# ariloytynoja/pagan2-msa

Hardware: AMD Instinct MI355X
Metric: DP cells/sec, 32x100 kb DNA progressive align (hot path in dependency order: fill + traceback per tree level) (higher is better)
Workload: dtype f64; 1 GPU; cfg4_32x100kb_dna_anchored; leaves=32, length=100000, data_type=dna, anchors=prefix, offset 15, node_alignments=31, order=guide-tree levels one after the other (a parent needs its children)

## Files before the change

### pagan2-msa_amd/csrc/dp_pipe.hip

```cpp
#include "dp_kcommon.h"
#include <type_traits>

#define PNW 4
#define PNT (64 * PNW)
#define PNTW PG_PIPE_WIDTH
#define PRK PG_PIPE_RING
#define PAGE PG_PIPE_REACH
#define PRW 512
#define PEC PG_PIPE_EDGE_CAP
#define PDR 128
#define PDR_REACH 60
#define PLOOK 64
#define PLAND 8
#define PNA PG_PIPE_ASSIST
#define PST PG_PIPE_STAGE
#define PBLOCK (PNT + 64 * PNA + 64)
static_assert(PNTW == PNT - PAGE && PRK >= PAGE && PG_PIPE_WINDOW + 80 <= PRW, "kernel geometry out of step with dp_device.h");
static_assert(PNA == 3 && PST == 3 && PAGE >= PLAND + 4, "assist wave a stages the diagonals d % 3 == a into slot a, at most two diagonals ahead; far cells have landed");
#define PFAR_POOL ((PNT * 4) / 24)
#define PS_ONLY 0x80000000u
#define PS_FIRST 0x40000000u
#define PS_BP 0x3fffffffu
#ifndef PG_SPIN_LIMIT_LOG2
#define PG_SPIN_LIMIT_LOG2 25
// ... 2002 lines not shown
            l2q[q] = r2q[q] = lSq[q] = rSq[q] = false;
            int kL = 0, kR = 0;
            gl[q] = pg_i4{0, 0, 0, 0}; gr[q] = pg_i4{0, 0, 0, 0};
#pragma unroll
            for (int t = 0; t < 8; ++t) { o_f[q][t].need = false; o_f[q][t].boff = 0; o_xy[q][t].x = NIw; o_xy[q][t].y = NIw; o_m[q][t] = NIw; }
            if (!__any(r <= hi)) continue;
            if (r <= hi) {
                gl[q] = PM.recL[r & (PRW - 1)]; gr[q] = PM.recR[j & (PRW - 1)];
                const int nl = (gl[q].x >> PR_NE_SHIFT) & 127, nr = (gr[q].x >> PR_NE_SHIFT) & 127;
                const int dl0 = gl[q].y & 0xffff, dl1 = (int)((unsigned)gl[q].y >> 16), dr0 = gr[q].y & 0xffff, dr1 = (int)((unsigned)gr[q].y >> 16);
                const bool easyL = nl == 1 ? dl0 == 1 : (nl == 2 && (dl0 == 1) != (dl1 == 1));
                const bool easyR = nr == 1 ? dr0 == 1 : (nr == 2 && (dr0 == 1) != (dr1 == 1));
                const bool l2 = nl == 2, r2 = nr == 2;
                const bool lS = l2 && dl0 != 1, rS = r2 && dr0 != 1;
                kL = lS ? dl0 : dl1; kR = rS ? dr0 : dr1;
                const bool inner = r >= 2 && r <= Lx - 2 && j >= 2 && j <= Ly - 2 && (!l2 || r - kL >= 1) && (!r2 || j - kR >= 1);
                kind[q] = (easyL && easyR && inner) ? 1 : 2;
                if (kind[q] == 1) { l2q[q] = l2; r2q[q] = r2; lSq[q] = lS; rSq[q] = rS; }
            }
            const bool b1 = kind[q] == 1, l2 = l2q[q], r2 = r2q[q];
            if (!__any(b1 && (l2 || r2))) continue;
            auto rd = [&](bool need, int age, int p_, pg_d2 &xy, double &m) {
                int rb = wsb - age * wrow_bytes;
                rb += rb < 0 ? wk * wrow_bytes : 0;
                const int off = need ? rb + wpos(p_) * 24 : (int)offsetof(PipeSmem, null_cell) - (int)offsetof(PipeSmem, sc);
                const double *c = (const double *)((const char *)&PM.sc[0][0][0] + off);
                xy.x = c[PG_X]; xy.y = c[PG_Y]; m = c[PG_M];
            };
            auto fetch = [&](int t, bool need, int age, int p_) {
                if (!__any(need)) return;
                if (!__any(need && age > amax)) rd(need, age, p_, o_xy[q][t], o_m[q][t]);
                else { o_f[q][t] = wcell(need, age, p_, o_xy[q][t], o_m[q][t]); any_far = true; }
            };
            fetch(3, b1 && l2, kL, r - kL);
            fetch(4, b1 && l2, kL + 1, r - kL);
            fetch(5, b1 && r2, kR, r);
            fetch(6, b1 && r2, kR + 1, r - 1);
            fetch(7, b1 && l2 && r2, kL + kR, r - kL);
        }
#ifdef PG_PIPE_STATS
        const long long st_t2 = __builtin_readcyclecounter();
#endif
        if (any_far) {
            far_fetch8(sc_out, o_f[0], o_xy[0], o_m[0]);
            far_fetch8(sc_out, o_f[1], o_xy[1], o_m[1]);
        }
#ifdef PG_PIPE_STATS
        const long long st_t3 = __builtin_readcyclecounter();
#endif
#pragma unroll
        for (int q = 0; q < 2; ++q) {
            const int r = wrow[q], j = d - r;
            const bool active = kind[q] != 0;
            if (__any(active)) n_now += 2;
            double bx = NIw, by = NIw, bm = NIw;
            unsigned px = PG_BP_NONE, py = PG_BP_NONE, pm = PG_BP_NONE;
            if (kind[q] == 1) {
                const bool l2 = l2q[q], r2 = r2q[q], lS = lSq[q], rS = rSq[q];
                const int ti_ = ((gl[q].x & 0xffff) + __umul24(gr[q].x & 0xffff, S)) & 255;
                const double tM = PM.tab2[ti_][0], tX = PM.tab2[ti_][1];
                const double lw0 = (double)__int_as_float(gl[q].z), lw1 = (double)__int_as_float(gl[q].w);
                const double rw0 = (double)__int_as_float(gr[q].z), rw1 = (double)__int_as_float(gr[q].w);
                const double lwA = lS ? lw1 : lw0, lwS = lS ? lw0 : lw1, rwA = rS ? rw1 : rw0, rwS = rS ? rw0 : rw1;
                const pg_d2 lx_ = o_xy[q][3], lm_ = o_xy[q][4], ry_ = o_xy[q][5], rm_ = o_xy[q][6], lr_ = o_xy[q][7];
                const double lxm = o_m[q][3], lmm = o_m[q][4], rym = o_m[q][5], rmm = o_m[q][6], lrm = o_m[q][7];
                auto gapv = [&](double own, double other, double m_) { return __builtin_fmax(own + ge, __builtin_fmax(other, m_ + ng) + go); };
                auto pairv = [&](double x_, double y_, double m_, double lw, double rw) {
                    return (__builtin_fmax(m_ + tM, __builtin_fmax(x_, y_) + tX) + lw) + rw;
                };
                bx = gapv(Ux[q], Uy[q], Um[q]);
                by = gapv(Py[q], Px[q], Pm[q]);
                bm = pairv(Cx[q], Cy[q], Cm[q], lwA, rwA);
                if (__any(r2)) {
                    by = __builtin_fmax(by, gapv(ry_.y, ry_.x, rym));
                    bm = __builtin_fmax(bm, pairv(rm_.x, rm_.y, rmm, lwA, rwS));
                }
                if (__any(l2)) {
                    bx = __builtin_fmax(bx, gapv(lx_.x, lx_.y, lxm));
                    bm = __builtin_fmax(bm, pairv(lm_.x, lm_.y, lmm, lwS, rwA));
                    if (__any(l2 && r2)) bm = __builtin_fmax(bm, pairv(lr_.x, lr_.y, lrm, lwS, rwS));
                }
            } else if (kind[q] == 2) {
                const int nl = (gl[q].x >> PR_NE_SHIFT) & 127, nr = (gr[q].x >> PR_NE_SHIFT) & 127;
                double tM_ = 0, tX_ = 0;
                if (r > 0 && j > 0 && nl > 0 && nr > 0) {
                    const int ti_ = ((gl[q].x & 0xffff) + __umul24(gr[q].x & 0xffff, S)) & 255;
                    tM_ = PM.tab2[ti_][0]; tX_ = PM.tab2[ti_][1];
                }
                const pg_i4 gl_ = gl[q], gr_ = gr[q];
                cell_any_t(J, r, j, r > 0 ? nl : 0, j > 0 ? nr : 0, tM_, tX_, no_terminal_edges, reduced_terminal,
                         [&](int p_, int q_, double &xs, double &ys, double &ms) {
                             pg_d2 xy; double m_;
                             const FarAsk f = wcell(p_ >= 0 && q_ >= 0, d - (p_ + q_), p_, xy, m_);
                             {
                                 const FarAsk none = {false, 0};
                                 pg_d2 e1 = {NIw, NIw}, e2 = {NIw, NIw}, e3 = {NIw, NIw}; double m1 = NIw, m2 = NIw, m3 = NIw;
                                 far_fetch4(sc_out, f, none, none, none, xy, m_, e1, m1, e2, m2, e3, m3);
                             }
                             xs = xy.x; ys = xy.y; ms = m_;
                         },
                         [&](int k, int &p_, double &lw) { int dist; edge_at<true>(gl_, k, r, dist, lw); p_ = r - dist; },
                         [&](int k, int &q_, double &rw) { int dist; edge_at<false>(gr_, k, j, dist, rw); q_ = j - dist; },
                         bx, by, bm, px, py, pm);
            }
            if (__any(active && ((gl[q].x | gr[q].x) & PR_SRC))) { if (active) hist_append(gl[q], gr[q], r, j, bx, by, bm); }
            if (r < lo + wpos_n) {
                double *o = (double *)((char *)&PM.sc[0][0][0] + wsb + wpos(r) * 24);
                o[PG_X] = bx; o[PG_Y] = by; o[PG_M] = bm;
            }
            if (active) {
                const unsigned off24 = __umul24((unsigned)(r - lo), 24u);
                pg_d2 xy; xy.x = bx; xy.y = by;
                *(PG_GLOBAL pg_d2 *)(srow + off24) = xy;
                *(PG_GLOBAL double *)(srow + off24 + 16u) = bm;
            }
            Px[q] = bx; Py[q] = by; Pm[q] = bm;
            Cx[q] = Ux[q]; Cy[q] = Uy[q]; Cm[q] = Um[q];
        }
        {
            const int tot = n_now + n_hist1 + n_hist2;
            if (tot >= 12) asm volatile("s_waitcnt vmcnt(12)" ::: "memory");
            else if (tot >= 10) asm volatile("s_waitcnt vmcnt(10)" ::: "memory");
            else if (tot >= 8) asm volatile("s_waitcnt vmcnt(8)" ::: "memory");
            else if (tot >= 6) asm volatile("s_waitcnt vmcnt(6)" ::: "memory");
            else if (tot >= 4) asm volatile("s_waitcnt vmcnt(4)" ::: "memory");
            else if (tot >= 2) asm volatile("s_waitcnt vmcnt(2)" ::: "memory");
            else asm volatile("s_waitcnt vmcnt(0)" ::: "memory");
            n_hist2 = n_hist1; n_hist1 = n_now;
        }
        flag_store(&PM.progress[wave], d);
#ifdef PG_PIPE_STATS
        {
            const long long st_t5 = __builtin_readcyclecounter();
            st_cls_t[4] += st_t5 - st_step0; ++st_cls_n[4];
            st_w[0] += st_t1 - st_step0; st_w[1] += st_t2 - st_t1; st_w[2] += st_t3 - st_t2; st_w[3] += st_t5 - st_t3;
        }
#endif
        ++d;
        lo_prev = lo;
        if (d >= run_end || flag_load(&PM.abort_flag) != 0) break;
        cur.x = __builtin_amdgcn_readfirstlane(nxt.x); cur.y = __builtin_amdgcn_readfirstlane(nxt.y);
        cur.z = __builtin_amdgcn_readfirstlane(nxt.z); cur.w = __builtin_amdgcn_readfirstlane(nxt.w);
    }
    dA = psc[d];
    row = dA.x + ((tid - dA.x) & (PNT - 1));
    ok_until = d - 1;
    C_.dA = dA;
    WCTX_OUT(C_);
}

#define PW7 7
#define PW7L (64 * PW7)
static_assert(PW7 == PNW + PNA && PG_PIPE_WINDOW <= PW7L - 16, "seven-wave wide runs: one row per lane");
__device__ __noinline__ void wide_run7(WaveCtx &C_) {
    WCTX_IN(C_);
    WCTX_STATS(C_);
    const PgDevJob *__restrict__ job = (const PgDevJob *)uniform_u64((unsigned long long)C_.job);
    const unsigned flags_ = __builtin_amdgcn_readfirstlane(C_.flags);
    const bool no_terminal_edges = flags_ & 1u, reduced_terminal = !(flags_ & 2u);
    pg_i8 dA = uniform_i8(C_.dA);
    const View J = load_view(job);
    const int d0 = d;
    const int lane = tid & 63, w7 = wave, up7 = w7 == 0 ? PW7 - 1 : w7 - 1;
    const double NIw = neg_inf();
    asm volatile("s_waitcnt vmcnt(0)" ::: "memory");
    flag_store(&PM.wflag[w7], d0 - 1);
    flag_store(&PM.warrived[w7], d0);
    for (int w = 0; w < PW7; ++w) POLLX(&PM.warrived[w], d0, 7);
    p_up = d0 - 1 > p_up ? d0 - 1 : p_up;
    p_dn = d0 - 1 > p_dn ? d0 - 1 : p_dn;
    int run_end = d0 + 1;
    for (;;) {
        const int t = run_end + lane;
        const int c4 = ((PG_GLOBAL const int *)psc)[8 * (t < nd ? t : nd) + 4] & 15;
        const unsigned long long stop = __builtin_amdgcn_ballot_w64(t >= nd || c4 != 4);
        if (stop != 0) { run_end += __builtin_ctzll(stop); break; }
        run_end += 64;
    }
    asm volatile("s_waitcnt vmcnt(0)" ::: "memory");
    pg_i4 cur = {dA.x, dA.y, dA.z, dA.w};
    int wr;
    { int m_ = (tid - cur.x) % PW7L; m_ += m_ < 0 ? PW7L : 0; wr = cur.x + m_; }
    if (diags_ld < d0) diags_ld = POLLX(&PM.loaded[2], d0, 5);
    double Px, Py, Pm, Cx, Cy, Cm, Ux, Uy, Um;
    {
        const FarAsk fP = far_ask(psc, d0, 1, wr), fC = far_ask(psc, d0, 2, wr - 1), fU = far_ask(psc, d0, 1, wr - 1), none = {false, 0};
        pg_d2 a = {NIw, NIw}, b = {NIw, NIw}, c = {NIw, NIw}, e = {NIw, NIw};
        double ma = NIw, mb = NIw, mc = NIw, me = NIw;
        far_fetch4(sc_out, fP, fC, fU, none, a, ma, b, mb, c, mc, e, me);
        Px = a.x; Py = a.y; Pm = ma; Cx = b.x; Cy = b.y; Cm = mb; Ux = c.x; Uy = c.y; Um = mc;
    }
    const bool geo_b = (dA.s4 & 16) != 0;
    const int wpos_n = geo_b ? PWPOS_B : PWPOS_A, wk = geo_b ? PWK_B : PWK_A, wage = wk - 2, wrow_bytes = wpos_n * 24;
    int wbase = cur.x - 32;
    auto wpos = [&](int r_) { int q_ = r_ - wbase; q_ -= q_ >= wpos_n ? wpos_n : 0; q_ -= q_ >= wpos_n ? wpos_n : 0; return q_; };
    int n_hist1 = 0, n_hist2 = 0;
    int lo_prev = cur.x;
    for (;;) {
        const int lo = cur.x, hi = cur.y;
        if (lo - 2 * wage - 4 - wbase >= wpos_n) wbase += wpos_n;
#ifdef PG_PIPE_STATS
        const long long st_step0 = __builtin_readcyclecounter();
#endif
        {
            const int nr_ = hi + 1 < Lx ? hi + 1 : Lx, nc_ = d - lo + 1 < Ly ? d - lo + 1 : Ly;
            if (rows_ld < nr_) rows_ld = POLLX(&PM.loaded[0], nr_, 1);
            if (cols_ld < nc_) cols_ld = POLLX(&PM.loaded[1], nc_, 2);
            if (diags_ld < d) diags_ld = POLLX(&PM.loaded[2], d, 5);
        }
        const int r = wr < lo ? wr + PW7L : wr, j = d - r;
        int kind = 0;
        pg_i4 gl = {0, 0, 0, 0}, gr = {0, 0, 0, 0};
        bool l2 = false, r2 = false, l3 = false, r3 = false;
        int kL = 1, kR = 1, kL3 = 1, kR3 = 1;
        double lwA = 0, lwS = 0, lwT = 0, rwA = 0, rwS = 0, rwT = 0;
        double tM = 0, tX = 0;
        if (r <= hi) {
            gl = PM.recL[r & (PRW - 1)]; gr = PM.recR[j & (PRW - 1)];
            const int nl = (gl.x >> PR_NE_SHIFT) & 127, nr = (gr.x >> PR_NE_SHIFT) & 127;
            auto shape = [&](auto left_tag, const pg_i4 &rec, int site, int n, bool &two, bool &three, int &k1, int &k3, double &wA, double &w1, double &w3) -> bool {
                constexpr bool LEFT = decltype(left_tag)::value;
                const int e0 = rec.y & 0xffff, e1 = (int)((unsigned)rec.y >> 16);
                const double f0 = (double)__int_as_float(rec.z), f1 = (double)__int_as_float(rec.w);
                two = false; three = false; k1 = 1; k3 = 1; wA = f0; w1 = 0.0; w3 = 0.0;
                if (n == 1) return e0 == 1;
                if (n == 2) {
                    two = true;
                    if (e0 == 1) { wA = f0; k1 = e1; w1 = f1; } else { wA = f1; k1 = e0; w1 = f0; }
                    return (e0 == 1) != (e1 == 1);
                }
                if (n == 3) {
                    int e2; double f2;
                    edge_at<LEFT>(rec, 2, site, e2, f2);
                    two = true; three = true;
                    if (e0 == 1) { wA = f0; k1 = e1; w1 = f1; k3 = e2; w3 = f2; }
                    else if (e1 == 1) { wA = f1; k1 = e0; w1 = f0; k3 = e2; w3 = f2; }
                    else { wA = f2; k1 = e0; w1 = f0; k3 = e1; w3 = f1; }
                    return ((e0 == 1) + (e1 == 1) + (e2 == 1)) == 1;
                }
                return false;
            };
            bool l2_, l3_, r2_, r3_;
            const bool easyL = shape(std::true_type(), gl, r, nl, l2_, l3_, kL, kL3, lwA, lwS, lwT);
            const bool easyR = shape(std::false_type(), gr, j, nr, r2_, r3_, kR, kR3, rwA, rwS, rwT);
            const bool inner = r >= 2 && r <= Lx - 2 && j >= 2 && j <= Ly - 2 && r - kL >= 1 && j - kR >= 1 && r - kL3 >= 1 && j - kR3 >= 1;
            kind = (easyL && easyR && inner && !(l3_ && r3_)) ? 1 : 2;
            if (kind == 1) { l2 = l2_; r2 = r2_; l3 = l3_; r3 = r3_; }
            if (r > 0 && j > 0 && nl > 0 && nr > 0) {
                const int ti_ = ((gl.x & 0xffff) + __umul24(gr.x & 0xffff, S)) & 255;
                tM = PM.tab2[ti_][0]; tX = PM.tab2[ti_][1];
            }
        }
        if (diags_ld < d + 2 && d + 1 < nd) diags_ld = POLLX(&PM.loaded[2], d + 2, 5);
        const pg_i4 nxt = PM.dring[(d + 1) & (PDR - 1)];
        const int amax = d - d0 < wage ? d - d0 : wage;
        const int wsb = (d % wk) * wrow_bytes;
        const long long soff = ((long long)cur.w << 32) | (unsigned)cur.z;
        PG_GLOBAL char *srow = (PG_GLOBAL char *)sc_out + soff;
        {
            int spins = 0;
            for (;;) {
                const int v = lane < PW7 ? flag_peek(&PM.wflag[lane]) : 0x7fffffff;
                if (__builtin_amdgcn_ballot_w64(v < (lane == up7 ? d - 1 : d - 2)) == 0) break;
                if ((++spins & 15) == 0) {
                    __builtin_amdgcn_s_sleep(1);
                    if (spins > PSPIN_LIMIT || flag_load(&PM.abort_flag) != 0) {
                        if (flag_load(&PM.abort_flag) == 0) flag_store(&PM.abort_flag, PTAG(6));
                        break;
                    }
                }
            }
        }
#ifdef PG_PIPE_STATS
        const long long st_t1 = __builtin_readcyclecounter();
#endif
#ifdef PG_EXP_WIDE_SKIP
        if (true) {
            flag_store(&PM.wflag[w7], d);
            if (w7 < PNW) flag_store(&PM.progress[w7], d);
            ++d; lo_prev = lo;
            if (d >= run_end || flag_load(&PM.abort_flag) != 0) break;
            cur.x = __builtin_amdgcn_readfirstlane(nxt.x); cur.y = __builtin_amdgcn_readfirstlane(nxt.y);
            cur.z = __builtin_amdgcn_readfirstlane(nxt.z); cur.w = __builtin_amdgcn_readfirstlane(nxt.w);
            continue;
        }
#endif
        if (d > d0) {
            int rb1 = wsb - wrow_bytes;
            rb1 += rb1 < 0 ? wk * wrow_bytes : 0;
            const double *c = (const double *)((const char *)&PM.sc[0][0][0] + rb1 + wpos(wr - 1) * 24);
            const double ax = dpp_shr1(Px, c[PG_X]), ay = dpp_shr1(Py, c[PG_Y]), am = dpp_shr1(Pm, c[PG_M]);
            const bool top = wr == lo_prev;
            Ux = top ? NIw : ax; Uy = top ? NIw : ay; Um = top ? NIw : am;
            if (wr < lo) { wr += PW7L; Px = NIw; Py = NIw; Pm = NIw; Cx = NIw; Cy = NIw; Cm = NIw; Ux = NIw; Uy = NIw; Um = NIw; }
        }
        auto wcell = [&](bool need, int age, int p_, pg_d2 &xy, double &m) -> FarAsk {
            FarAsk f = {false, 0};
            xy.x = NIw; xy.y = NIw; m = NIw;
            if (!need || (age == 1 && d > d0 && p_ < lo_prev)) return f;
            if (age <= amax) {
                int rb = wsb - age * wrow_bytes;
                rb += rb < 0 ? wk * wrow_bytes : 0;
                const double *c = (const double *)((const char *)&PM.sc[0][0][0] + rb + wpos(p_) * 24);
                xy.x = c[PG_X]; xy.y = c[PG_Y]; m = c[PG_M];
                return f;
            }
            return far_ask(psc, d, age, p_);
        };
        pg_d2 o_xy[8];
        double o_m[8];
        FarAsk o_f[8];
        bool any_far = false;
#pragma unroll
        for (int t = 0; t < 8; ++t) { o_f[t].need = false; o_f[t].boff = 0; o_xy[t].x = NIw; o_xy[t].y = NIw; o_m[t] = NIw; }
        const bool b1 = kind == 1;
        if (__any(b1 && (l2 || r2))) {
            auto rd = [&](bool need, int age, int p_, pg_d2 &xy, double &m) {
                int rb = wsb - age * wrow_bytes;
                rb += rb < 0 ? wk * wrow_bytes : 0;
                const int off = need ? rb + wpos(p_) * 24 : (int)offsetof(PipeSmem, null_cell) - (int)offsetof(PipeSmem, sc);
                const double *c = (const double *)((const char *)&PM.sc[0][0][0] + off);
                xy.x = c[PG_X]; xy.y = c[PG_Y]; m = c[PG_M];
            };
            auto fetch = [&](int t, bool need, int age, int p_) {
                if (!__any(need)) return;
                if (!__any(need && age > amax)) rd(need, age, p_, o_xy[t], o_m[t]);
                else { o_f[t] = wcell(need, age, p_, o_xy[t], o_m[t]); any_far = true; }
            };
            fetch(3, b1 && l2, kL, r - kL);
            fetch(4, b1 && l2, kL + 1, r - kL);
            fetch(5, b1 && r2, kR, r);
            fetch(6, b1 && r2, kR + 1, r - 1);
            fetch(7, b1 && l2 && r2, kL + kR, r - kL);
        }
#ifdef PG_PIPE_STATS
        const long long st_t2 = __builtin_readcyclecounter();
#endif
        if (any_far) far_fetch8(sc_out, o_f, o_xy, o_m);
#ifdef PG_PIPE_STATS
        const long long st_t3 = __builtin_readcyclecounter();
#endif
        const bool active = kind != 0;
        const int n_now = __any(active) ? 2 : 0;
        double bx = NIw, by = NIw, bm = NIw;
        unsigned px = PG_BP_NONE, py = PG_BP_NONE, pm = PG_BP_NONE;
        if (kind == 1) {
            const pg_d2 lx_ = o_xy[3], lm_ = o_xy[4], ry_ = o_xy[5], rm_ = o_xy[6], lr_ = o_xy[7];
            const double lxm = o_m[3], lmm = o_m[4], rym = o_m[5], rmm = o_m[6], lrm = o_m[7];
            auto gapv = [&](double own, double other, double m_) { return __builtin_fmax(own + ge, __builtin_fmax(other, m_ + ng) + go); };
            auto pairv = [&](double x_, double y_, double m_, double lw, double rw) {
                return (__builtin_fmax(m_ + tM, __builtin_fmax(x_, y_) + tX) + lw) + rw;
            };
            bx = gapv(Ux, Uy, Um);
            by = gapv(Py, Px, Pm);
            bm = pairv(Cx, Cy, Cm, lwA, rwA);
            if (__any(r2)) {
                by = __builtin_fmax(by, gapv(ry_.y, ry_.x, rym));
                bm = __builtin_fmax(bm, pairv(rm_.x, rm_.y, rmm, lwA, rwS));
            }
            if (__any(l2)) {
                bx = __builtin_fmax(bx, gapv(lx_.x, lx_.y, lxm));
                bm = __builtin_fmax(bm, pairv(lm_.x, lm_.y, lmm, lwS, rwA));
                if (__any(l2 && r2)) bm = __builtin_fmax(bm, pairv(lr_.x, lr_.y, lrm, lwS, rwS));
            }
            if (__any(l3 || r3)) {
                const bool t3 = l3 || r3;
                const int k3 = l3 ? kL3 : kR3;
                const bool needC = l3 ? r2 : (r3 && l2);
                pg_d2 txy[3]; double tm_[3];
                const FarAsk fA = wcell(t3, k3, l3 ? r - kL3 : r, txy[0], tm_[0]);
                const FarAsk fB = wcell(t3, k3 + 1, l3 ? r - kL3 : r - 1, txy[1], tm_[1]);
                const FarAsk fC = wcell(needC, l3 ? kL3 + kR : kL + kR3, l3 ? r - kL3 : r - kL, txy[2], tm_[2]);
                {
                    const FarAsk none = {false, 0};
                    pg_d2 e = {NIw, NIw}; double me = NIw;
                    far_fetch4(sc_out, fA, fB, fC, none, txy[0], tm_[0], txy[1], tm_[1], txy[2], tm_[2], e, me);
                }
                if (l3) {
                    bx = __builtin_fmax(bx, gapv(txy[0].x, txy[0].y, tm_[0]));
                    bm = __builtin_fmax(bm, pairv(txy[1].x, txy[1].y, tm_[1], lwT, rwA));
                    bm = __builtin_fmax(bm, pairv(txy[2].x, txy[2].y, tm_[2], lwT, rwS));
                } else if (r3) {
                    by = __builtin_fmax(by, gapv(txy[0].y, txy[0].x, tm_[0]));
                    bm = __builtin_fmax(bm, pairv(txy[1].x, txy[1].y, tm_[1], lwA, rwT));
                    bm = __builtin_fmax(bm, pairv(txy[2].x, txy[2].y, tm_[2], lwS, rwT));
                }
            }
        } else if (kind == 2) {
            const int nl = (gl.x >> PR_NE_SHIFT) & 127, nr = (gr.x >> PR_NE_SHIFT) & 127;
            const pg_i4 gl_ = gl, gr_ = gr;
            cell_any_t(J, r, j, r > 0 ? nl : 0, j > 0 ? nr : 0, tM, tX, no_terminal_edges, reduced_terminal,
                     [&](int p_, int q_, double &xs, double &ys, double &ms) {
                         pg_d2 xy; double m_;
                         const FarAsk f = wcell(p_ >= 0 && q_ >= 0, d - (p_ + q_), p_, xy, m_);
                         {
                             const FarAsk none = {false, 0};
                             pg_d2 e1 = {NIw, NIw}, e2 = {NIw, NIw}, e3 = {NIw, NIw}; double m1 = NIw, m2 = NIw, m3 = NIw;
                             far_fetch4(sc_out, f, none, none, none, xy, m_, e1, m1, e2, m2, e3, m3);
                         }
                         xs = xy.x; ys = xy.y; ms = m_;
                     },
                     [&](int k, int &p_, double &lw) { int dist; edge_at<true>(gl_, k, r, dist, lw); p_ = r - dist; },
                     [&](int k, int &q_, double &rw) { int dist; edge_at<false>(gr_, k, j, dist, rw); q_ = j - dist; },
                     bx, by, bm, px, py, pm);
        }
        if (wr < lo + wpos_n) {
            double *o = (double *)((char *)&PM.sc[0][0][0] + wsb + wpos(wr) * 24);
            o[PG_X] = bx; o[PG_Y] = by; o[PG_M] = bm;
        }
        if (__any(kind != 0 && ((gl.x | gr.x) & PR_SRC))) { if (kind != 0) hist_append(gl, gr, r, j, bx, by, bm); }
        if (wpos_n > PW7L && wr < lo + wpos_n - PW7L) {
            double *o = (double *)((char *)&PM.sc[0][0][0] + wsb + wpos(wr + PW7L) * 24);
            o[PG_X] = NIw; o[PG_Y] = NIw; o[PG_M] = NIw;
        }
        {
            const int tot = n_hist1 + n_hist2;
            if (tot >= 4) asm volatile("s_waitcnt vmcnt(4)" ::: "memory");
            else if (tot >= 2) asm volatile("s_waitcnt vmcnt(2)" ::: "memory");
            else asm volatile("s_waitcnt vmcnt(0)" ::: "memory");
            n_hist2 = n_hist1; n_hist1 = n_now;
        }
        flag_store(&PM.wflag[w7], d);
        if (w7 < PNW) flag_store(&PM.progress[w7], d);
        if (active) {
            const unsigned off24 = __umul24((unsigned)(wr - lo), 24u);
            pg_d2 xy; xy.x = bx; xy.y = by;
            *(PG_GLOBAL pg_d2 *)(srow + off24) = xy;
            *(PG_GLOBAL double *)(srow + off24 + 16u) = bm;
        }
        Px = bx; Py = by; Pm = bm;
        Cx = Ux; Cy = Uy; Cm = Um;
#ifdef PG_PIPE_STATS
        if (w7 < PNW) {
            const long long st_t5 = __builtin_readcyclecounter();
            st_cls_t[4] += st_t5 - st_step0; ++st_cls_n[4];
            st_w[0] += st_t1 - st_step0; st_w[1] += st_t2 - st_t1; st_w[2] += st_t3 - st_t2; st_w[3] += st_t5 - st_t3;
        }
#endif
        ++d;
        lo_prev = lo;
        if (d >= run_end || flag_load(&PM.abort_flag) != 0) break;
        cur.x = __builtin_amdgcn_readfirstlane(nxt.x); cur.y = __builtin_amdgcn_readfirstlane(nxt.y);
        cur.z = __builtin_amdgcn_readfirstlane(nxt.z); cur.w = __builtin_amdgcn_readfirstlane(nxt.w);
    }
    asm volatile("s_waitcnt vmcnt(0)" ::: "memory");
    flag_store(&PM.warrived[w7], d);
    for (int w = 0; w < PW7; ++w) POLLX(&PM.warrived[w], d, 7);
    dA = psc[d];
    row = dA.x + ((tid - dA.x) & (PNT - 1));
    ok_until = d - 1;
    C_.dA = dA;
    WCTX_OUT(C_);
}

__device__ __noinline__ void widest_run7(WaveCtx &C_) {
    WCTX_IN(C_);
    WCTX_STATS(C_);
    const PgDevJob *__restrict__ job = (const PgDevJob *)uniform_u64((unsigned long long)C_.job);
    const unsigned flags_ = __builtin_amdgcn_readfirstlane(C_.flags);
    const bool no_terminal_edges = flags_ & 1u, reduced_terminal = !(flags_ & 2u);
    pg_i8 dA = uniform_i8(C_.dA);
    const int d0 = d;
    const int lane = tid & 63, w7 = wave;
    asm volatile("s_waitcnt vmcnt(0)" ::: "memory");
    flag_store(&PM.wflag[w7], d0 - 1);
    flag_store(&PM.warrived[w7], d0);
    for (int w = 0; w < PW7; ++w) POLLX(&PM.warrived[w], d0, 7);
    p_up = d0 - 1 > p_up ? d0 - 1 : p_up;
    p_dn = d0 - 1 > p_dn ? d0 - 1 : p_dn;
    int run_end = d0 + 1;
    for (;;) {
        const int t = run_end + lane;
        const int c5 = ((PG_GLOBAL const int *)psc)[8 * (t < nd ? t : nd) + 4] & 15;
        const unsigned long long stop = __builtin_amdgcn_ballot_w64(t >= nd || c5 != 5);
        if (stop != 0) { run_end += __builtin_ctzll(stop); break; }
        run_end += 64;
    }
    asm volatile("s_waitcnt vmcnt(0)" ::: "memory");
    for (;;) {
        {
            int spins = 0;
            for (;;) {
                const int v = lane < PW7 ? flag_peek(&PM.wflag[lane]) : 0x7fffffff;
                if (__builtin_amdgcn_ballot_w64(v < d - 1) == 0) break;
                if ((++spins & 15) == 0) {
                    __builtin_amdgcn_s_sleep(1);
                    if (spins > PSPIN_LIMIT || flag_load(&PM.abort_flag) != 0) {
                        if (flag_load(&PM.abort_flag) == 0) flag_store(&PM.abort_flag, PTAG(6));
                        break;
                    }
                }
            }
        }
        const pg_i8 cur = psc[d];
#ifdef PG_PIPE_STATS
        const long long st_step0 = __builtin_readcyclecounter();
#endif
#ifndef PG_EXP_WIDEST_SKIP
        widest_step(job, psc, d, cur.x, cur.y, tid, no_terminal_edges, reduced_terminal, PW7L);
#endif
        flag_store(&PM.wflag[w7], d);
        if (w7 < PNW) flag_store(&PM.progress[w7], d);
#ifdef PG_PIPE_STATS
        if (w7 < PNW) { st_cls_t[4] += __builtin_readcyclecounter() - st_step0; ++st_cls_n[4]; }
#endif
        ++d;
        if (d >= run_end || flag_load(&PM.abort_flag) != 0) break;
    }
    asm volatile("s_waitcnt vmcnt(0)" ::: "memory");
    flag_store(&PM.warrived[w7], d);
    for (int w = 0; w < PW7; ++w) POLLX(&PM.warrived[w], d, 7);
    dA = psc[d];
    row = dA.x + ((tid - dA.x) & (PNT - 1));
    ok_until = d - 1;
    C_.dA = dA;
    WCTX_OUT(C_);
}

__device__ __noinline__ pg_i4 assist_wide_run(const PgDevJob *__restrict__ job, cdesc8_p psc, int a, int lane, unsigned flags, int d0,
                                              int rows_ld, int cols_ld, int diags_ld) {
    WaveCtx C_;
    C_.job = job; C_.psc = psc; C_.sc_out = (gdouble_w)job->sc; C_.bp_out = (gu32_w)job->bp;
    C_.go = (double)job->go; C_.ng = (double)job->ng; C_.ge = (double)job->ge; C_.tng2 = 0.0; C_.tng1 = 0.0;
    C_.Lx = job->Lx; C_.Ly = job->Ly; C_.nd = job->nd; C_.S = job->S; C_.sleep = job->nd;
    C_.tid = PNT + 64 * a + lane; C_.wave = PNW + a; C_.up = 0; C_.dn = 0; C_.bslot = 0; C_.flags = flags;
    C_.d = d0; C_.row = 0;
    C_.px = 0.0; C_.py = 0.0; C_.pm = 0.0; C_.cx = 0.0; C_.cy = 0.0; C_.cm = 0.0;
    C_.ca = pg_i4{0, 0, 0, 0}; C_.cb = pg_i4{0, 0, 0, 0}; C_.smf = 0.0f;
    C_.dA = psc[d0];
    C_.p_up = -1; C_.p_dn = -1; C_.ok_until = -1; C_.rows_ld = rows_ld; C_.cols_ld = cols_ld; C_.diags_ld = diags_ld;
    C_.as0 = 0; C_.as1 = 0; C_.as2 = 0;
#ifdef PG_PIPE_STATS
    for (int k = 0; k < 5; ++k) { C_.st_cls_t[k] = 0; C_.st_cls_n[k] = 0; }
    for (int k = 0; k < 10; ++k) { C_.st_poll_t[k] = 0; C_.st_poll_n[k] = 0; }
    for (int k = 0; k < 4; ++k) C_.st_w[k] = 0;
#endif
    if ((C_.dA.s4 & 15) == 5) widest_run7(C_); else wide_run7(C_);
    return pg_i4{C_.d, C_.rows_ld, C_.cols_ld, C_.diags_ld};
}

#ifdef PG_PIPE_STATS
#ifndef PG_STAT_CLASS
#define PG_STAT_CLASS 0
#endif
#define PSTAMP(k) do { const long long t_ = __builtin_readcyclecounter(); if (st_on) st_acc[k] += t_ - st_t; st_t = t_; } while (0)
#else
#define PSTAMP(k)
#endif

__device__ __forceinline__ int peek_l2(PG_GLOBAL const int *p) {
    int v;
    asm volatile("global_load_dword %0, %1, off sc1\n\ts_waitcnt vmcnt(0)" : "=&v"(v) : "v"(p) : "memory");
    return __builtin_amdgcn_readfirstlane(v);
}
__device__ __forceinline__ unsigned my_xcc_id() {
    unsigned x;
    asm volatile("s_getreg_b32 %0, hwreg(HW_REG_XCC_ID)" : "=s"(x));
    return x & 15u;
}

__device__ __noinline__ void follow_chunk(const PgDevJob *__restrict__ job, int chunk, int lane, unsigned flags) {
    const View J = load_view(job);
    const bool no_terminal_edges = flags & 1u;
    const bool reduced_terminal = !(flags & 2u);
    const int first = chunk * PG_FOLLOW_CHUNK, end = first + PG_FOLLOW_CHUNK < J.nd ? first + PG_FOLLOW_CHUNK : J.nd;
    for (int d = first; d < end; ++d) {
        const pg_i4 cur = J.dsc[d];
        const int lo = cur.x, hi = cur.y;
        if (hi < lo) continue;
        const long long base = ((long long)cur.w << 32) | (unsigned)cur.z;
        Diag d1 = {0, -1, 0}, d2 = {0, -1, 0};
        if (d > 0) { const pg_i4 p = J.dsc[d - 1]; d1 = {p.x, p.y, ((long long)p.w << 32) | (unsigned)p.z}; }
        if (d > 1) { const pg_i4 p = J.dsc[d - 2]; d2 = {p.x, p.y, ((long long)p.w << 32) | (unsigned)p.z}; }
        for (int i = lo + lane; i <= hi; i += 64) {
            const int j = d - i;
            const long long at = base + (i - lo);
            int l0 = 0, l1 = 0, r0 = 0, r1 = 0;
            if (i > 0) { l0 = J.offL[i]; l1 = J.offL[i + 1]; }
            if (j > 0) { r0 = J.offR[j]; r1 = J.offR[j + 1]; }
            float sm = 0.0f;
            if (i > 0 && j > 0 && l1 > l0 && r1 > r0) sm = J.table[J.stL[i] + J.stR[j] * J.S];
            double bx, by, bm;
            unsigned px, py, pm;
            cell_any(J, i, j, l1 - l0, r1 - r0, sm, no_terminal_edges, reduced_terminal,
                     [&](int p, int q, double &xs, double &ys, double &ms) {
                         const long long ix = hbm_index(J, d, d1, d2, p, q);
                         xs = ys = ms = neg_inf();
                         if (ix >= 0) far_cell((PG_GLOBAL const double *)(J.sc + 3 * ix), xs, ys, ms);
                     },
                     [&](int k, int &p, double &lw) { p = J.srcL[l0 + k]; lw = (double)J.lwL[l0 + k]; },
                     [&](int k, int &q, double &rw) { q = J.srcR[r0 + k]; rw = (double)J.lwR[r0 + k]; },
                     bx, by, bm, px, py, pm);
// ... 587 lines not shown
```

Measured before the change: 592.7 million cells/s.

## Cache left-site shape per row and issue far fetches before the wave wait

In the seven-wave wide run, the left record and its edge shape are now decoded only when a lane's row changes, not on every diagonal. Window offsets (wsb, wqb) are carried incrementally instead of recomputed with modulo each step. Operand addresses are planned before the inter-wave spin wait, and global far-cell loads are issued there so their latency overlaps the wait. The cost is more live registers (five cached three-double operands), and it relies on new PR_TWO/PR_THREE flags in the records.

Result: faster. 606.4 million cells/s, median of 6 (+2.3%).

```diff
diff --git a/pagan2-msa_amd/csrc/dp_pipe.hip b/pagan2-msa_amd/csrc/dp_pipe.hip
--- a/pagan2-msa_amd/csrc/dp_pipe.hip
+++ b/pagan2-msa_amd/csrc/dp_pipe.hip
@@ -2178,6 +2178,41 @@
 #define PW7 7
 #define PW7L (64 * PW7)
 static_assert(PW7 == PNW + PNA && PG_PIPE_WINDOW <= PW7L - 16, "seven-wave wide runs: one row per lane");
+template <bool LEFT>
+__device__ __forceinline__ bool site7(const pg_i4 &rec, int site, bool &two, bool &three, int &k1, int &k3, double &wA, double &w1, double &w3) {
+    const int n = (rec.x >> PR_NE_SHIFT) & 127;
+    two = false; three = false; k1 = 1; k3 = 1; wA = (double)__int_as_float(rec.z); w1 = 0.0; w3 = 0.0;
+    if (rec.x & PR_TWO) {
+        two = true; k1 = (int)((unsigned)rec.y >> 16); w1 = (double)__int_as_float(rec.w);
+        if (rec.x & PR_THREE) { three = true; edge_at<LEFT>(rec, 2, site, k3, w3); }
+        return true;
+    }
+    if (n == 1) return (rec.y & 0xffff) == 1;
+    if (n == 3) {
+        const int e0 = rec.y & 0xffff, e1 = (int)((unsigned)rec.y >> 16);
+        const double f0 = wA, f1 = (double)__int_as_float(rec.w);
+        int e2; double f2;
+        edge_at<LEFT>(rec, 2, site, e2, f2);
+        two = true; three = true;
+        if (e0 == 1) { k1 = e1; w1 = f1; k3 = e2; w3 = f2; }
+        else if (e1 == 1) { wA = f1; k1 = e0; w1 = f0; k3 = e2; w3 = f2; }
+        else { wA = f2; k1 = e0; w1 = f0; k3 = e1; w3 = f1; }
+        return ((e0 == 1) + (e1 == 1) + (e2 == 1)) == 1;
+    }
+    return false;
+}
+__device__ __forceinline__ void far_issue(gdouble_w sc, const FarAsk &a, unsigned long long (&q)[3]) {
+#ifdef PG_PIPE_STATS
+    const bool bad = a.need && (a.boff < 0 || a.boff + 24 > PM.far_limit);
+    if (__builtin_amdgcn_ballot_w64(bad) != 0 && PM.abort_flag == 0) PM.abort_flag = 0x7f000005;
+    PG_GLOBAL const unsigned long long *p = (PG_GLOBAL const unsigned long long *)((PG_GLOBAL const char *)sc + (a.need && !bad ? a.boff : 0ll));
+#else
+    PG_GLOBAL const unsigned long long *p = (PG_GLOBAL const unsigned long long *)((PG_GLOBAL const char *)sc + (a.need ? a.boff : 0ll));
+#endif
+    q[0] = __hip_atomic_load(p, __ATOMIC_RELAXED, __HIP_MEMORY_SCOPE_AGENT);
+    q[1] = __hip_atomic_load(p + 1, __ATOMIC_RELAXED, __HIP_MEMORY_SCOPE_AGENT);
+    q[2] = __hip_atomic_load(p + 2, __ATOMIC_RELAXED, __HIP_MEMORY_SCOPE_AGENT);
+}
 __device__ __noinline__ void wide_run7(WaveCtx &C_) {
     WCTX_IN(C_);
     WCTX_STATS(C_);
@@ -2222,6 +2257,13 @@
     auto wpos = [&](int r_) { int q_ = r_ - wbase; q_ -= q_ >= wpos_n ? wpos_n : 0; q_ -= q_ >= wpos_n ? wpos_n : 0; return q_; };
     int n_hist1 = 0, n_hist2 = 0;
     int lo_prev = cur.x;
+    const int wring_bytes = wk * wrow_bytes;
+    int wsb = (d0 % wk) * wrow_bytes;
+    int wqb = wpos(wr) * 24;
+    int lrow = -1, lbits = 0;
+    pg_i4 gl = {0, 0, 0, 0};
+    int kL = 1, kL3 = 1;
+    double lwA = 0, lwS = 0, lwT = 0;
     for (;;) {
         const int lo = cur.x, hi = cur.y;
         if (lo - 2 * wage - 4 - wbase >= wpos_n) wbase += wpos_n;
@@ -2235,54 +2277,70 @@
             if (diags_ld < d) diags_ld = POLLX(&PM.loaded[2], d, 5);
         }
         const int r = wr < lo ? wr + PW7L : wr, j = d - r;
+        if (__any(r <= hi && r != lrow)) {
+            if (r <= hi && r != lrow) {
+                lrow = r;
+                gl = PM.recL[r & (PRW - 1)];
+                bool two, three;
+                const bool easy = site7<true>(gl, r, two, three, kL, kL3, lwA, lwS, lwT);
+                const bool in = r >= 2 && r <= Lx - 2 && r - kL >= 1 && r - kL3 >= 1;
+                lbits = (easy && in ? 1 : 0) | (two ? 2 : 0) | (three ? 4 : 0) | (r > 0 && ((gl.x >> PR_NE_SHIFT) & 127) > 0 ? 8 : 0);
+            }
+        }
         int kind = 0;
-        pg_i4 gl = {0, 0, 0, 0}, gr = {0, 0, 0, 0};
-        bool l2 = false, r2 = false, l3 = false, r3 = false;
-        int kL = 1, kR = 1, kL3 = 1, kR3 = 1;
-        double lwA = 0, lwS = 0, lwT = 0, rwA = 0, rwS = 0, rwT = 0;
+        pg_i4 gr = {0, 0, 0, 0};
+        bool r2_ = false, r3_ = false;
+        int kR = 1, kR3 = 1;
+        double rwA = 0, rwS = 0, rwT = 0;
         double tM = 0, tX = 0;
         if (r <= hi) {
-            gl = PM.recL[r & (PRW - 1)]; gr = PM.recR[j & (PRW - 1)];
-            const int nl = (gl.x >> PR_NE_SHIFT) & 127, nr = (gr.x >> PR_NE_SHIFT) & 127;
-            auto shape = [&](auto left_tag, const pg_i4 &rec, int site, int n, bool &two, bool &three, int &k1, int &k3, double &wA, double &w1, double &w3) -> bool {
-                constexpr bool LEFT = decltype(left_tag)::value;
-                const int e0 = rec.y & 0xffff, e1 = (int)((unsigned)rec.y >> 16);
-                const double f0 = (double)__int_as_float(rec.z), f1 = (double)__int_as_float(rec.w);
-                two = false; three = false; k1 = 1; k3 = 1; wA = f0; w1 = 0.0; w3 = 0.0;
-                if (n == 1) return e0 == 1;
-                if (n == 2) {
-                    two = true;
-                    if (e0 == 1) { wA = f0; k1 = e1; w1 = f1; } else { wA = f1; k1 = e0; w1 = f0; }
-                    return (e0 == 1) != (e1 == 1);
-                }
-                if (n == 3) {
-                    int e2; double f2;
-                    edge_at<LEFT>(rec, 2, site, e2, f2);
-                    two = true; three = true;
-                    if (e0 == 1) { wA = f0; k1 = e1; w1 = f1; k3 = e2; w3 = f2; }
-                    else if (e1 == 1) { wA = f1; k1 = e0; w1 = f0; k3 = e2; w3 = f2; }
-                    else { wA = f2; k1 = e0; w1 = f0; k3 = e1; w3 = f1; }
-                    return ((e0 == 1) + (e1 == 1) + (e2 == 1)) == 1;
-                }
-                return false;
-            };
-            bool l2_, l3_, r2_, r3_;
-            const bool easyL = shape(std::true_type(), gl, r, nl, l2_, l3_, kL, kL3, lwA, lwS, lwT);
-            const bool easyR = shape(std::false_type(), gr, j, nr, r2_, r3_, kR, kR3, rwA, rwS, rwT);
-            const bool inner = r >= 2 && r <= Lx - 2 && j >= 2 && j <= Ly - 2 && r - kL >= 1 && j - kR >= 1 && r - kL3 >= 1 && j - kR3 >= 1;
-            kind = (easyL && easyR && inner && !(l3_ && r3_)) ? 1 : 2;
-            if (kind == 1) { l2 = l2_; r2 = r2_; l3 = l3_; r3 = r3_; }
-            if (r > 0 && j > 0 && nl > 0 && nr > 0) {
+            gr = PM.recR[j & (PRW - 1)];
+            const bool easyR = site7<false>(gr, j, r2_, r3_, kR, kR3, rwA, rwS, rwT);
+            const bool in = j >= 2 && j <= Ly - 2 && j - kR >= 1 && j - kR3 >= 1;
+            kind = ((lbits & 1) && easyR && in && !((lbits & 4) && r3_)) ? 1 : 2;
+            if ((lbits & 8) && j > 0 && ((gr.x >> PR_NE_SHIFT) & 127) > 0) {
                 const int ti_ = ((gl.x & 0xffff) + __umul24(gr.x & 0xffff, S)) & 255;
                 tM = PM.tab2[ti_][0]; tX = PM.tab2[ti_][1];
             }
         }
+        const bool b1 = kind == 1;
+        const bool l2 = b1 && (lbits & 2), l3 = b1 && (lbits & 4), r2 = b1 && r2_, r3 = b1 && r3_;
         if (diags_ld < d + 2 && d + 1 < nd) diags_ld = POLLX(&PM.loaded[2], d + 2, 5);
         const pg_i4 nxt = PM.dring[(d + 1) & (PDR - 1)];
         const int amax = d - d0 < wage ? d - d0 : wage;
-        const int wsb = (d % wk) * wrow_bytes;
         const long long soff = ((long long)cur.w << 32) | (unsigned)cur.z;
         PG_GLOBAL char *srow = (PG_GLOBAL char *)sc_out + soff;
+        const int null_off = (int)offsetof(PipeSmem, null_cell) - (int)offsetof(PipeSmem, sc);
+        int o_off[5] = {null_off, null_off, null_off, null_off, null_off};
+        FarAsk o_f[5] = {{false, 0}, {false, 0}, {false, 0}, {false, 0}, {false, 0}};
+        bool o_any[5] = {false, false, false, false, false};
+        unsigned long long o_q[5][3];
+        bool any_far = false;
+        if (__any(l2 || r2)) {
+            auto plan = [&](int t, bool need, int age, int p_) {
+                if (!__any(need)) return;
+                o_any[t] = true;
+                if (need) {
+                    if (age <= amax) {
+                        int rb = wsb - age * wrow_bytes;
+                        rb += rb < 0 ? wring_bytes : 0;
+                        o_off[t] = rb + wpos(p_) * 24;
+                    } else o_f[t] = far_ask(psc, d, age, p_);
+                }
+            };
+            plan(0, l2, kL, r - kL);
+            plan(1, l2, kL + 1, r - kL);
+            plan(2, r2, kR, r);
+            plan(3, r2, kR + 1, r - 1);
+            plan(4, l2 && r2, kL + kR, r - kL);
+            any_far = __any(o_f[0].need || o_f[1].need || o_f[2].need || o_f[3].need || o_f[4].need);
+        }
+#if !defined(PG_WIDE7_FETCH_BEHIND) && !defined(PG_EXP_WIDE_SKIP)
+        if (any_far) {
+#pragma unroll
+            for (int t = 0; t < 5; ++t) far_issue(sc_out, o_f[t], o_q[t]);
+        }
+#endif
         {
             int spins = 0;
             for (;;) {
@@ -2305,6 +2363,7 @@
             flag_store(&PM.wflag[w7], d);
             if (w7 < PNW) flag_store(&PM.progress[w7], d);
             ++d; lo_prev = lo;
+            wsb += wrow_bytes; wsb = wsb == wring_bytes ? 0 : wsb;
             if (d >= run_end || flag_load(&PM.abort_flag) != 0) break;
             cur.x = __builtin_amdgcn_readfirstlane(nxt.x); cur.y = __builtin_amdgcn_readfirstlane(nxt.y);
             cur.z = __builtin_amdgcn_readfirstlane(nxt.z); cur.w = __builtin_amdgcn_readfirstlane(nxt.w);
@@ -2313,12 +2372,15 @@
 #endif
         if (d > d0) {
             int rb1 = wsb - wrow_bytes;
-            rb1 += rb1 < 0 ? wk * wrow_bytes : 0;
-            const double *c = (const double *)((const char *)&PM.sc[0][0][0] + rb1 + wpos(wr - 1) * 24);
+            rb1 += rb1 < 0 ? wring_bytes : 0;
+            const double *c = (const double *)((const char *)&PM.sc[0][0][0] + rb1 + (wqb != 0 ? wqb : wrow_bytes) - 24);
             const double ax = dpp_shr1(Px, c[PG_X]), ay = dpp_shr1(Py, c[PG_Y]), am = dpp_shr1(Pm, c[PG_M]);
             const bool top = wr == lo_prev;
             Ux = top ? NIw : ax; Uy = top ? NIw : ay; Um = top ? NIw : am;
-            if (wr < lo) { wr += PW7L; Px = NIw; Py = NIw; Pm = NIw; Cx = NIw; Cy = NIw; Cm = NIw; Ux = NIw; Uy = NIw; Um = NIw; }
+            if (wr < lo) {
+                wqb += PW7L * 24; wqb -= wqb >= wrow_bytes ? wrow_bytes : 0; wqb -= wqb >= wrow_bytes ? wrow_bytes : 0;
+                wr += PW7L; Px = NIw; Py = NIw; Pm = NIw; Cx = NIw; Cy = NIw; Cm = NIw; Ux = NIw; Uy = NIw; Um = NIw;
+            }
         }
         auto wcell = [&](bool need, int age, int p_, pg_d2 &xy, double &m) -> FarAsk {
             FarAsk f = {false, 0};
@@ -2333,36 +2395,29 @@
             }
             return far_ask(psc, d, age, p_);
         };
-        pg_d2 o_xy[8];
-        double o_m[8];
-        FarAsk o_f[8];
-        bool any_far = false;
+        pg_d2 o_xy[5];
+        double o_m[5];
 #pragma unroll
-        for (int t = 0; t < 8; ++t) { o_f[t].need = false; o_f[t].boff = 0; o_xy[t].x = NIw; o_xy[t].y = NIw; o_m[t] = NIw; }
-        const bool b1 = kind == 1;
-        if (__any(b1 && (l2 || r2))) {
-            auto rd = [&](bool need, int age, int p_, pg_d2 &xy, double &m) {
-                int rb = wsb - age * wrow_bytes;
-                rb += rb < 0 ? wk * wrow_bytes : 0;
-                const int off = need ? rb + wpos(p_) * 24 : (int)offsetof(PipeSmem, null_cell) - (int)offsetof(PipeSmem, sc);
-                const double *c = (const double *)((const char *)&PM.sc[0][0][0] + off);
-                xy.x = c[PG_X]; xy.y = c[PG_Y]; m = c[PG_M];
-            };
-            auto fetch = [&](int t, bool need, int age, int p_) {
-                if (!__any(need)) return;
-                if (!__any(need && age > amax)) rd(need, age, p_, o_xy[t], o_m[t]);
-                else { o_f[t] = wcell(need, age, p_, o_xy[t], o_m[t]); any_far = true; }
-            };
-            fetch(3, b1 && l2, kL, r - kL);
-            fetch(4, b1 && l2, kL + 1, r - kL);
-            fetch(5, b1 && r2, kR, r);
-            fetch(6, b1 && r2, kR + 1, r - 1);
-            fetch(7, b1 && l2 && r2, kL + kR, r - kL);
+        for (int t = 0; t < 5; ++t) {
+            o_xy[t].x = NIw; o_xy[t].y = NIw; o_m[t] = NIw;
+            if (o_any[t]) {
+                const double *c = (const double *)((const char *)&PM.sc[0][0][0] + o_off[t]);
+                o_xy[t].x = c[PG_X]; o_xy[t].y = c[PG_Y]; o_m[t] = c[PG_M];
+            }
         }
 #ifdef PG_PIPE_STATS
         const long long st_t2 = __builtin_readcyclecounter();
 #endif
-        if (any_far) far_fetch8(sc_out, o_f, o_xy, o_m);
+        if (any_far) {
+#ifdef PG_WIDE7_FETCH_BEHIND
+#pragma unroll
+            for (int t = 0; t < 5; ++t) far_issue(sc_out, o_f[t], o_q[t]);
+#endif
+#pragma unroll
+            for (int t = 0; t < 5; ++t) {
+                if (o_f[t].need) { o_xy[t].x = __longlong_as_double((long long)o_q[t][0]); o_xy[t].y = __longlong_as_double((long long)o_q[t][1]); o_m[t] = __longlong_as_double((long long)o_q[t][2]); }
+            }
+        }
 #ifdef PG_PIPE_STATS
         const long long st_t3 = __builtin_readcyclecounter();
 #endif
@@ -2371,8 +2426,8 @@
         double bx = NIw, by = NIw, bm = NIw;
         unsigned px = PG_BP_NONE, py = PG_BP_NONE, pm = PG_BP_NONE;
         if (kind == 1) {
-            const pg_d2 lx_ = o_xy[3], lm_ = o_xy[4], ry_ = o_xy[5], rm_ = o_xy[6], lr_ = o_xy[7];
-            const double lxm = o_m[3], lmm = o_m[4], rym = o_m[5], rmm = o_m[6], lrm = o_m[7];
+            const pg_d2 lx_ = o_xy[0], lm_ = o_xy[1], ry_ = o_xy[2], rm_ = o_xy[3], lr_ = o_xy[4];
+            const double lxm = o_m[0], lmm = o_m[1], rym = o_m[2], rmm = o_m[3], lrm = o_m[4];
             auto gapv = [&](double own, double other, double m_) { return __builtin_fmax(own + ge, __builtin_fmax(other, m_ + ng) + go); };
             auto pairv = [&](double x_, double y_, double m_, double lw, double rw) {
                 return (__builtin_fmax(m_ + tM, __builtin_fmax(x_, y_) + tX) + lw) + rw;
@@ -2431,12 +2486,13 @@
                      bx, by, bm, px, py, pm);
         }
         if (wr < lo + wpos_n) {
-            double *o = (double *)((char *)&PM.sc[0][0][0] + wsb + wpos(wr) * 24);
+            double *o = (double *)((char *)&PM.sc[0][0][0] + wsb + wqb);
             o[PG_X] = bx; o[PG_Y] = by; o[PG_M] = bm;
         }
         if (__any(kind != 0 && ((gl.x | gr.x) & PR_SRC))) { if (kind != 0) hist_append(gl, gr, r, j, bx, by, bm); }
         if (wpos_n > PW7L && wr < lo + wpos_n - PW7L) {
-            double *o = (double *)((char *)&PM.sc[0][0][0] + wsb + wpos(wr + PW7L) * 24);
+            int q_ = wqb + PW7L * 24; q_ -= q_ >= wrow_bytes ? wrow_bytes : 0;
+            double *o = (double *)((char *)&PM.sc[0][0][0] + wsb + q_);
             o[PG_X] = NIw; o[PG_Y] = NIw; o[PG_M] = NIw;
         }
         {
@@ -2464,6 +2520,7 @@
         }
 #endif
         ++d;
+        wsb += wrow_bytes; wsb = wsb == wring_bytes ? 0 : wsb;
         lo_prev = lo;
         if (d >= run_end || flag_load(&PM.abort_flag) != 0) break;
         cur.x = __builtin_amdgcn_readfirstlane(nxt.x); cur.y = __builtin_amdgcn_readfirstlane(nxt.y);
```
